# inferflow/inferflow

Measured on AMD Instinct MI355X. Metric: decode tokens/sec, Llama-2-7B Q4 batch=1 greedy (whole job), higher is better.
Workload: dtype i8 (Q8 activations x Q4_B32T1A weights, i32 dot, f32 scale, f16 I/O); 1 GPU; llama2_7b decode, Q4_B32T1A weights + F16 lm_head, F16 KV cache, batch 1 greedy, 16-token prompt, context 21..1851; parallelism=single, weights_bytes=4309647360

## Files before the change

### inferflow_amd/csrc/ifa_decode_attn.h

```cpp
#pragma once
#include "ifa_decode_kernels.h"

namespace ifa {

struct DecAttnParams {
    const half_t *q;
    const half_t *k_new;
    const half_t *v_new;
    uint8_t *kcache, *vcache;
    const int *state;
    const float *rope_tab;
    int heads, kv_heads, kv_q8;
    float kq_scale;
    int rope_order, rope_cols;
    int alibi, alibi_base, alibi_total;
    half_t *out;
    int max_ctx;
    int8_t *xq;
    long long *trace;
    const void *batch_rows;
    int q_stride;
};
struct DecAttnBatchRow { const uint8_t *kc, *vc; int n_ctx, pad; };

// ... 49 lines not shown
        if constexpr (IFA_ATTN_NACC == 1) return c[0];
        else if constexpr (IFA_ATTN_NACC == 2) return c[0] + c[1];
        else if constexpr (IFA_ATTN_NACC == 4) return (c[0] + c[1]) + (c[2] + c[3]);
        else { float t = c[0]; for (int i = 1; i < IFA_ATTN_NACC; i++) t = t + c[i]; return t; }
    }
};

struct DecAttnFusedIn {
    const unsigned long long *gran;
    unsigned epoch;
    int pos;
    unsigned *err;
    long long timeout_ticks;
    unsigned long long *att_gran;
};

__host__ __device__ inline int att_gran_count(int heads, int hd) { return heads * hd / 4 + 2 * (heads * hd / 32) + heads; }

template <int HD, bool Q8, int PB, bool KT>
struct DecAttnRegs {
    static constexpr int DG = HD / 8, NSPLIT = 256 / DG, VPRE = PB / NSPLIT;
    static constexpr int KBYTES = (HD / 32) * 34;
    static constexpr int KALIGN = HD == 128 ? 8 : (HD == 64 ? 4 : 2);
    uint32_t kreg[Q8 ? 1 : HD / 2];
    uint32_t kq32[(Q8 && KALIGN >= 4) ? KBYTES / 4 : 1];
    uint16_t kq16[(Q8 && KALIGN < 4) ? KBYTES / 2 : 1];
    u32x4 kt[KT ? PB / NSPLIT : 1];
    u32x4 vreg[Q8 ? 1 : VPRE];
    uint32_t vqs[Q8 ? VPRE : 1], vqc[Q8 ? VPRE : 1][2];
    float rope_cs, rope_sn;
    half_t q_in, k_in, v_in;
};

template <int HD, bool Q8, bool BATCH, int PB, bool KT, bool FUSED, int PHASE = 0>
__device__ __forceinline__ void dec_attn_body(char *smem, const half_t *pq, const uint8_t *pkc, const uint8_t *pvc, int pheads, int pkvh,
                                              const DecAttnParams &P, const int h_in, const DecAttnFusedIn &F, DecAttnRegs<HD, Q8, PB, KT> &R)
{
    int pos_b = 0;
    if constexpr (FUSED) pos_b = F.pos;
    if constexpr (BATCH) {
        const DecAttnBatchRow br = reinterpret_cast<const DecAttnBatchRow *>(P.batch_rows)[blockIdx.y];
        pkc = br.kc; pvc = br.vc; pos_b = br.n_ctx - 1;
        pq += (size_t)blockIdx.y * P.q_stride;
    }
#define IFA_GP(T, p) ((const __attribute__((address_space(1))) T *)(p))
    uint8_t *const kcw = BATCH ? const_cast<uint8_t *>(pkc) : P.kcache;
    uint8_t *const vcw = BATCH ? const_cast<uint8_t *>(pvc) : P.vcache;
    const float *const rope_tab = BATCH ? P.rope_tab + (size_t)blockIdx.y * HD : P.rope_tab;
    half_t *const outp = BATCH ? P.out + (size_t)blockIdx.y * pheads * HD : P.out;
    static_assert(HD % 8 == 0 && HD <= 128 && (!Q8 || HD % 32 == 0), "head size: multiples of 8 up to 128 (Q8 rows: whole 32-blocks)");
    constexpr int DG = HD / 8;
    constexpr int NSPLIT = 256 / DG;
    half_t *qs = reinterpret_cast<half_t *>(smem);
    half_t *kn = qs + HD;
    half_t *vn = kn + HD;
    float *red = reinterpret_cast<float *>(vn + HD);
    float *opart = red + 16;
    static_assert(!KT || (!Q8 && !BATCH && (DG & (DG - 1)) == 0 && PB % NSPLIT == 0), "K tile through LDS: F16 rows, one query, power-of-two pieces per row");
    static_assert(!(FUSED && BATCH), "the fused tail is a single-query kernel");
    static_assert(PB >= NSPLIT && PB <= DEC_ATTN_MIN_ROWS, "prefetch bucket");
    uint8_t *ktile = reinterpret_cast<uint8_t *>(opart + NSPLIT * HD);
    half_t *S = reinterpret_cast<half_t *>(ktile + (KT ? (size_t)PB * HD * 2 : 0));
    const int h = h_in, tid = threadIdx.x, lane = tid & 63, wave = tid >> 6;
    const int group = pheads / pkvh;
    const int kvh = h / group;
    const bool writer = (h % group) == 0;
    const int kv_dim = pkvh * HD;
    const size_t row_bytes = Q8 ? (size_t)(kv_dim / 32) * 34 : (size_t)kv_dim * 2;
    const size_t head_off = Q8 ? (size_t)((kvh * HD) / 32) * 34 : (size_t)kvh * HD * 2;

    constexpr int KBYTES = (HD / 32) * 34;
    constexpr int KALIGN = HD == 128 ? 8 : (HD == 64 ? 4 : 2);
    auto &kreg = R.kreg; auto &kq32 = R.kq32; auto &kq16 = R.kq16; auto &kt = R.kt; auto &vreg = R.vreg; auto &vqs = R.vqs; auto &vqc = R.vqc;
    float &rope_cs = R.rope_cs, &rope_sn = R.rope_sn;
    half_t &q_in = R.q_in, &k_in = R.k_in, &v_in = R.v_in;
    auto load_k = [&](int j) {
        const uint8_t *rowp = pkc + (size_t)j * row_bytes + head_off;
        if constexpr (Q8) {
            if constexpr (KALIGN == 8) {
#pragma unroll
                for (int i = 0; i < KBYTES / 8; i++) {
                    const u32x2 t = IFA_GP(u32x2, rowp)[i];
                    kq32[2 * i] = t[0]; kq32[2 * i + 1] = t[1];
                }
            } else if constexpr (KALIGN == 4) {
#pragma unroll
                for (int i = 0; i < KBYTES / 4; i++) kq32[i] = IFA_GP(uint32_t, rowp)[i];
            } else {
#pragma unroll
                for (int i = 0; i < KBYTES / 2; i++) kq16[i] = IFA_GP(uint16_t, rowp)[i];
            }
        } else {
#pragma unroll
            for (int i = 0; i < HD / 8; i++) {
                const u32x4 t = IFA_GP(u32x4, rowp)[i];
                kreg[4 * i] = t[0]; kreg[4 * i + 1] = t[1]; kreg[4 * i + 2] = t[2]; kreg[4 * i + 3] = t[3];
            }
        }
    };
    auto kbyte = [&](int B) -> uint32_t {
        if constexpr (KALIGN >= 4) return (kq32[B >> 2] >> (8 * (B & 3))) & 0xFFu;
        else return (kq16[B >> 1] >> (8 * (B & 1))) & 0xFFu;
    };
    const int dq = min(tid, HD - 1);
    if constexpr (PHASE != 2) {
    q_in = (half_t)0; k_in = (half_t)0; v_in = (half_t)0;
    if constexpr (!FUSED) { q_in = pq[(size_t)h * HD + dq]; k_in = pq[(size_t)(pheads + kvh) * HD + dq]; v_in = pq[(size_t)(pheads + pkvh + kvh) * HD + dq]; }
    }
    const int dg = tid % DG, sp = tid / DG;
    const bool vact = (256 % DG == 0) || sp < NSPLIT;
    constexpr int VPRE = PB / NSPLIT;
    if constexpr (PHASE != 2) {
    if constexpr (KT) {
#pragma unroll
        for (int i = 0; i < PB / NSPLIT; i++) kt[i] = IFA_GP(u32x4, pkc + (size_t)min(sp + NSPLIT * i, FUSED ? min(pos_b, PB - 1) : PB - 1) * row_bytes + head_off)[dg];
    } else {
        load_k((BATCH || FUSED) ? min(tid, min(pos_b, PB - 1)) : min(tid, PB - 1));
    }
    rope_cs = 1.0f; rope_sn = 0.0f;
    {
        const int c = min(tid < HD / 2 ? tid : tid - HD / 2, HD / 2 - 1);
        const float *rt = rope_tab ? rope_tab : reinterpret_cast<const float *>(pq);
        typedef float f32x2 __attribute__((ext_vector_type(2)));
        const f32x2 cs = *IFA_GP(f32x2, rt + 2 * c);
        if (P.rope_order != 0) { rope_cs = cs[0]; rope_sn = cs[1]; }
    }
    const size_t vq_off = head_off + (size_t)(dg / 4) * 34;
#pragma unroll
    for (int i = 0; i < VPRE; i++) {
        const int j = min(sp + NSPLIT * i, BATCH ? pos_b : (FUSED ? min(pos_b, PB - 1) : PB - 1));
        if constexpr (!Q8) {
            vreg[i] = IFA_GP(u32x4, pvc + (size_t)j * row_bytes + head_off)[dg];
        } else {
            const auto *blk = IFA_GP(uint16_t, pvc + (size_t)j * row_bytes + vq_off);
            typedef uint32_t u32x2_a2 __attribute__((ext_vector_type(2), aligned(2)));
            vqs[i] = blk[0];
            const u32x2_a2 cw = *IFA_GP(u32x2_a2, blk + 1 + (dg % 4) * 4);
            vqc[i][0] = cw[0]; vqc[i][1] = cw[1];
        }
    }
    }
    if constexpr (PHASE == 1) return;

    const bool tr = P.trace != nullptr && tid == 0;
    if (tr) P.trace[h * 8 + 0] = wall_clock64();
    const int pos = (BATCH || FUSED) ? pos_b : *(const __attribute__((address_space(4))) int *)(P.state + 1);
    const int n_ctx = pos + 1;
    if constexpr (FUSED) {
        if (tid < HD) {
            const unsigned long long *gq = F.gran + (size_t)h * HD + tid, *gk = F.gran + (size_t)(pheads + kvh) * HD + tid,
                                     *gv = F.gran + (size_t)(pheads + pkvh + kvh) * HD + tid;
            const long long t_give_up = wall_clock64() + F.timeout_ticks;
            for (;;) {
                const unsigned long long a = __hip_atomic_load(gq, __ATOMIC_RELAXED, __HIP_MEMORY_SCOPE_AGENT);
                const unsigned long long b = __hip_atomic_load(gk, __ATOMIC_RELAXED, __HIP_MEMORY_SCOPE_AGENT);
                const unsigned long long c = __hip_atomic_load(gv, __ATOMIC_RELAXED, __HIP_MEMORY_SCOPE_AGENT);
                const bool ok = (unsigned)(a >> 32) == F.epoch && (unsigned)(b >> 32) == F.epoch && (unsigned)(c >> 32) == F.epoch;
                q_in = __builtin_bit_cast(half_t, (uint16_t)a); k_in = __builtin_bit_cast(half_t, (uint16_t)b); v_in = __builtin_bit_cast(half_t, (uint16_t)c);
                if (__all(ok)) break;
                if (wall_clock64() > t_give_up) { if (lane == 0) atomicExch(F.err, 0x51u); break; }
                __builtin_amdgcn_s_sleep(2);
            }
        }
    }
    if (tid < HD) { qs[tid] = q_in; kn[tid] = k_in; vn[tid] = v_in; }
    if constexpr (KT) {
#pragma unroll
        for (int i = 0; i < PB / NSPLIT; i++) {
            const int j = sp + NSPLIT * i;
            *reinterpret_cast<u32x4 *>(ktile + ((size_t)j * DG + (size_t)(dg ^ (j & (DG - 1)))) * 16) = kt[i];
        }
    }
    __syncthreads();
    if (tr) P.trace[h * 8 + 1] = wall_clock64();
    if (P.rope_order != 0) {
        if (tid < HD) {
            const int c = tid < HD / 2 ? tid : tid - HD / 2;
            rope_apply(tid < HD / 2 ? qs : kn, c, rope_cs, rope_sn, P.rope_order, P.rope_cols);
        }
        __syncthreads();
    }
// ... 160 lines not shown
    __syncthreads();
    }
    if (tr) P.trace[h * 8 + 5] = wall_clock64();

    float o[8];
#pragma unroll
    for (int i = 0; i < 8; i++) o[i] = 0.0f;
    auto acc_v = [&](float pj, const u32x4 vv) {
        const half8_t v8 = __builtin_bit_cast(half8_t, vv);
#pragma unroll
        for (int e = 0; e < 8; e++) o[e] = __builtin_fmaf(pj, (float)v8[e], o[e]);
    };
    auto acc_new = [&](float pj) {
#pragma unroll
        for (int e = 0; e < 8; e++) o[e] = __builtin_fmaf(pj, h2f(vn[dg * 8 + e]), o[e]);
    };
    auto acc_q8w = [&](float pj, uint16_t scb, uint16_t c0, uint16_t c1, uint16_t c2, uint16_t c3) {
        const half_t sch = __builtin_bit_cast(half_t, scb);
        const half2_t sc2 = {sch, sch};
        half2_t v01, v23, v45, v67;
        q8x4_dequant_h((uint32_t)c0 | ((uint32_t)c1 << 16), sc2, v01, v23);
        q8x4_dequant_h((uint32_t)c2 | ((uint32_t)c3 << 16), sc2, v45, v67);
        o[0] = __builtin_fmaf(pj, (float)v01[0], o[0]); o[1] = __builtin_fmaf(pj, (float)v01[1], o[1]);
        o[2] = __builtin_fmaf(pj, (float)v23[0], o[2]); o[3] = __builtin_fmaf(pj, (float)v23[1], o[3]);
        o[4] = __builtin_fmaf(pj, (float)v45[0], o[4]); o[5] = __builtin_fmaf(pj, (float)v45[1], o[5]);
        o[6] = __builtin_fmaf(pj, (float)v67[0], o[6]); o[7] = __builtin_fmaf(pj, (float)v67[1], o[7]);
    };
    auto acc_q8 = [&](float pj, int j) {
        const auto *blk = IFA_GP(uint16_t, pvc + (size_t)j * row_bytes + head_off + (size_t)(dg / 4) * 34);
        typedef uint32_t u32x2_a2 __attribute__((ext_vector_type(2), aligned(2)));
        const u32x2_a2 cw = *IFA_GP(u32x2_a2, blk + 1 + (dg % 4) * 4);
        acc_q8w(pj, blk[0], (uint16_t)(cw[0] & 0xFFFFu), (uint16_t)(cw[0] >> 16), (uint16_t)(cw[1] & 0xFFFFu), (uint16_t)(cw[1] >> 16));
    };
#pragma unroll
    for (int i = 0; i < VPRE; i++) {
        const int j = sp + NSPLIT * i;
        if (j < n_ctx && vact) {
            const float pj = h2f(S[j]);
            if (j == pos) acc_new(pj);
            else if constexpr (Q8) acc_q8w(pj, (uint16_t)vqs[i], (uint16_t)(vqc[i][0] & 0xFFFFu), (uint16_t)(vqc[i][0] >> 16), (uint16_t)(vqc[i][1] & 0xFFFFu), (uint16_t)(vqc[i][1] >> 16));
            else acc_v(pj, vreg[i]);
        }
    }
    {
        constexpr int TB = 8;
        u32x4 tcur[Q8 ? 1 : TB], tnxt[Q8 ? 1 : TB];
        uint32_t ts_c[Q8 ? TB : 1], tc_c[Q8 ? TB : 1][2], ts_n[Q8 ? TB : 1], tc_n[Q8 ? TB : 1][2];
        const size_t tq_off = head_off + (size_t)(dg / 4) * 34;
        auto tload = [&](u32x4 (&dst)[Q8 ? 1 : TB], uint32_t (&ds)[Q8 ? TB : 1], uint32_t (&dc)[Q8 ? TB : 1][2], int j) {
#pragma unroll
            for (int u = 0; u < TB; u++) {
                const int jr = min(j + u * NSPLIT, n_ctx - 1);
                if constexpr (!Q8) dst[u] = IFA_GP(u32x4, pvc + (size_t)jr * row_bytes + head_off)[dg];
                else {
                    const auto *blk = IFA_GP(uint16_t, pvc + (size_t)jr * row_bytes + tq_off);
                    typedef uint32_t u32x2_a2 __attribute__((ext_vector_type(2), aligned(2)));
                    ds[u] = blk[0];
                    const u32x2_a2 cw = *IFA_GP(u32x2_a2, blk + 1 + (dg % 4) * 4);
                    dc[u][0] = cw[0]; dc[u][1] = cw[1];
                }
            }
        };
        int j = vact ? sp + NSPLIT * VPRE : n_ctx;
        if (j < n_ctx) tload(tcur, ts_c, tc_c, j);
        for (; j < n_ctx; j += TB * NSPLIT) {
            tload(tnxt, ts_n, tc_n, j + TB * NSPLIT);
#pragma unroll
            for (int u = 0; u < TB; u++) {
                const int jj = j + u * NSPLIT;
                if (jj >= n_ctx) break;
                const float pj = h2f(S[jj]);
                if (jj == pos) acc_new(pj);
                else if constexpr (Q8) acc_q8w(pj, (uint16_t)ts_c[u], (uint16_t)(tc_c[u][0] & 0xFFFFu), (uint16_t)(tc_c[u][0] >> 16), (uint16_t)(tc_c[u][1] & 0xFFFFu), (uint16_t)(tc_c[u][1] >> 16));
                else acc_v(pj, tcur[u]);
            }
#pragma unroll
            for (int u = 0; u < TB; u++) {
                if constexpr (Q8) { ts_c[u] = ts_n[u]; tc_c[u][0] = tc_n[u][0]; tc_c[u][1] = tc_n[u][1]; }
                else tcur[u] = tnxt[u];
            }
        }
    }
    if (vact) {
#pragma unroll
        for (int e = 0; e < 8; e++) opart[sp * HD + dg * 8 + e] = o[e];
    }
    if (tr) P.trace[h * 8 + 6] = wall_clock64();
    __syncthreads();
    if (tid < HD) {
        float acc = opart[tid];
        for (int s2 = 1; s2 < NSPLIT; s2++) acc = acc + opart[s2 * HD + tid];
        const half_t yh = f2h(acc);
        outp[(size_t)h * HD + tid] = yh;
        if constexpr (HD % 32 == 0 && !BATCH) { if (P.xq) dec_attn_emit_q8<HD>(P.xq, P.heads * HD, h, tid, yh); }
        if constexpr (FUSED && HD % 32 == 0) {
            if (F.att_gran) {
                const float val = h2f(yh);
                const float mxv = half_wave_max(fabsf(val));
                const float qsc = mxv / 127;
                const int qv = q8_round_div1(val, qsc);
                const int sum = half_wave_sum_i32(qv);
                const int q1 = dpp_xor1(qv), q2 = dpp_xor2(qv), q3 = dpp_xor1(q2);
                const unsigned long long tagw = (unsigned long long)F.epoch << 32;
                const int cols = pheads * HD, nc = cols / 4, nbk = cols / 32;
                if ((tid & 3) == 0) {
                    const uint32_t w4 = (uint32_t)(qv & 0xFF) | ((uint32_t)(q1 & 0xFF) << 8) | ((uint32_t)(q2 & 0xFF) << 16) | ((uint32_t)(q3 & 0xFF) << 24);
                    __hip_atomic_store(F.att_gran + (h * HD + tid) / 4, tagw | w4, __ATOMIC_RELAXED, __HIP_MEMORY_SCOPE_AGENT);
                }
                if ((tid & 31) == 0) {
                    const int blk = (h * HD + tid) >> 5;
                    __hip_atomic_store(F.att_gran + nc + blk, tagw | __builtin_bit_cast(uint32_t, h2f(f2h(qsc))), __ATOMIC_RELAXED, __HIP_MEMORY_SCOPE_AGENT);
                    __hip_atomic_store(F.att_gran + nc + nbk + blk, tagw | __builtin_bit_cast(uint32_t, (float)sum), __ATOMIC_RELAXED, __HIP_MEMORY_SCOPE_AGENT);
                }
                if (tid == 0) __hip_atomic_store(F.att_gran + nc + 2 * nbk + h, tagw | 1u, __ATOMIC_RELAXED, __HIP_MEMORY_SCOPE_AGENT);
            }
        }
    }
    if (tr) P.trace[h * 8 + 7] = wall_clock64();
}

template <int HD, bool Q8, bool BATCH = false, int PB = DEC_ATTN_MIN_ROWS, bool KT = false>
__global__ void __launch_bounds__(256) k_dec_attn(const half_t *pq, const uint8_t *pkc, const uint8_t *pvc, int pheads, int pkvh,
                                                  const DecAttnParams P)
{
// ... 341 lines not shown
```

### inferflow_amd/csrc/ifa_decode_qkv_attn.h

```cpp
#pragma once
#include "ifa_decode_kernels.h"
#include "ifa_decode_attn.h"

namespace ifa {

struct DecQkvAttnExtra {
    unsigned long long *gran;
    const unsigned *epoch;
    unsigned epoch_add;
    unsigned *err;
    int timeout_us;
    int gk;
    int unload;
};

#ifndef IFA_QA_EARLY_KV
#define IFA_QA_EARLY_KV 0
#endif
#ifndef IFA_QA_WARM_ROWS
#define IFA_QA_WARM_ROWS 1
#endif
constexpr int QA_THREADS = 512;

template <int DT, int NJ, int RW, int NORM, int HD, bool Q8, int PB, bool KT, int NP, bool UL = false>
__global__ void __launch_bounds__(QA_THREADS) k_dec_qkv_attn(const half_t *px, const half_t *pnw, const half_t *pnb, int pcols, int pgeo,
                                                             const uint8_t *pwq, const uint8_t *pwk, const uint8_t *pwv,
                                                             const DecGemvParams P, const DecAttnParams A, const DecQkvAttnExtra E)
{
    const int g_heads = pgeo & 0xFF, g_kvh = (pgeo >> 8) & 0xFF, g_gk = (pgeo >> 16) & 0xFFFF;
    const int g_nblk = pcols / block_capacity(DT);
    extern __shared__ __attribute__((aligned(16))) char smem[];
    const long long t_kernel = wall_clock64();
    static_assert(NORM == 0 || NORM == 1, "QKV prologue: quantiser with or without the RMS norm");
    static_assert(NP > 0 && NP * 64 < QA_THREADS, "wave-specialised prologue");
    constexpr int TH = QA_THREADS, PT = NP * 64;
    constexpr int MAXC = (NJ * 8 * block_capacity(DT) + PT - 1) / PT;
    XPre<NORM, MAXC, false, PT> pre;
    if (threadIdx.x < PT) pre.issue(px, pnw, pnb, pcols);
    const XLds L = xlds_carve(smem, pcols);
    const int lane = threadIdx.x & 63;
    const int wave = __builtin_amdgcn_readfirstlane(threadIdx.x >> 6);
    using Fmt = DecFmt<DT, NJ>;
    const size_t row_bytes = tiled_row_bytes(DT, (size_t)g_nblk);
    const int g = (int)blockIdx.x / g_gk, bg = (int)blockIdx.x - g * g_gk;
    const int group = g_heads / g_kvh;
    const int RG = (group + 2) * HD;
    const int per = g_gk / group;
    const bool attn_wg = bg % per == 0;
    const int head = g * group + bg / per;
    const int WGV = UL ? (g_gk - group) * (TH / 64) : g_gk * (TH / 64);
    const int lw = UL ? (bg - bg / per - 1) * (TH / 64) + wave : bg * (TH / 64) + wave;
    struct Row { const uint8_t *w; const half_t *b; half_t *y; int row, vrow; };
    auto locate = [&](int lr) {
        Row r;
        const int nq = group * HD;
        const bool isk = lr >= nq && lr < nq + HD, isv = lr >= nq + HD;
        r.row = isv ? g * HD + (lr - nq - HD) : (isk ? g * HD + (lr - nq) : g * nq + lr);
// ... 27 lines not shown
    };
    static_assert(NP == 4, "the prologue waves are the attention waves");
    const bool ul_head = UL && attn_wg;
    if (!ul_head && threadIdx.x == TH - 1) { L.part[130] = 0.0f; L.part[131] = 0.0f; }
    if (!ul_head && wave >= NP) load_rows(0, 1);
    const int pos = *(const __attribute__((address_space(4))) int *)(A.state + 1);
    const unsigned epoch = ((*(const __attribute__((address_space(4))) unsigned *)(E.epoch) + E.epoch_add) << 20) | ((unsigned)pos & 0xFFFFFu);
    DecAttnFusedIn F;
    F.gran = E.gran; F.epoch = epoch; F.pos = pos; F.err = E.err; F.timeout_ticks = (long long)E.timeout_us * 100;
    F.att_gran = nullptr;
    if constexpr (UL) {
        if (attn_wg) {
            if (wave >= 4) {
#if IFA_QA_WARM_ROWS
                if (pos >= PB) {
                    constexpr int SB = Q8 ? (HD / 32) * 34 : HD * 2;
                    const int kvh = head / group, kv_dim = g_kvh * HD;
                    const size_t rb = Q8 ? (size_t)(kv_dim / 32) * 34 : (size_t)kv_dim * 2;
                    const size_t ho = Q8 ? (size_t)((kvh * HD) / 32) * 34 : (size_t)kvh * HD * 2;
                    const int t = (int)threadIdx.x - 256;
                    const int off = min((t & 3) * 64, SB - 4) & ~1;
                    typedef uint32_t u32_a2 __attribute__((aligned(2)));
                    uint32_t acc = 0;
                    for (int j = PB + (t >> 2); j <= pos; j += 64) {
                        acc ^= *(const __attribute__((address_space(1))) u32_a2 *)(A.kcache + (size_t)j * rb + ho + off);
                        acc ^= *(const __attribute__((address_space(1))) u32_a2 *)(A.vcache + (size_t)j * rb + ho + off);
                    }
                    if (acc == 0x9E3779B9u && A.trace) A.trace[(size_t)A.heads * 8 + 7] = (long long)acc;
                }
#endif
                return;
            }
            DecAttnRegs<HD, Q8, PB, KT> RU;
            dec_attn_body<HD, Q8, false, PB, KT, true>(smem, nullptr, A.kcache, A.vcache, A.heads, A.kv_heads, A, head, F, RU);
            return;
        }
    }
    __syncthreads();
    DecAttnRegs<HD, Q8, PB, KT> R;
    if (wave >= NP) {
        load_rows(1, RW);
    } else {
        pre.finish(P.norm_w, P.norm_b, P.multi_base, P.eps, P.cols, L, P.xn_out, nullptr);
        load_rows(0, RW);
#if IFA_QA_EARLY_KV
        if (attn_wg) dec_attn_body<HD, Q8, false, PB, KT, true, 1>(smem, nullptr, A.kcache, A.vcache, A.heads, A.kv_heads, A, head, F, R);
#endif
    }
    lds_counter_wait(L.part + 131, NP);
    typename Fmt::X X;
    X.load(L.codes, L.scale, L.xsum, lane, g_nblk);
    {
        float a[RW];
#pragma unroll
        for (int i = 0; i < RW; i++) a[i] = w[i].dot(X);
#pragma unroll
        for (int i = 0; i < RW; i++) a[i] = wave_sum(a[i]);
        float a0 = 0.0f;
#pragma unroll
        for (int i = 0; i < RW; i++) { if (lane == i) a0 = a[i]; }
        const int lr = lane * WGV + lw;
        if (lane < RW && lr < RG) {
            const Row r = locate(lr);
            half_t y = dec_bias(a0, r.b, r.row);
            if (P.pre_scale != 0.0f) y = f2h(h2f(y) * P.pre_scale);
            r.y[r.row] = y;
            __hip_atomic_store(E.gran + r.vrow, ((unsigned long long)epoch << 32) | (unsigned long long)__builtin_bit_cast(uint16_t, y),
                               __ATOMIC_RELAXED, __HIP_MEMORY_SCOPE_AGENT);
        }
    }
    if (A.trace && threadIdx.x == 0) {
        A.trace[(size_t)(A.heads + (int)blockIdx.x) * 8 + 0] = t_kernel;
        A.trace[(size_t)(A.heads + (int)blockIdx.x) * 8 + 1] = wall_clock64();
    }
    if (attn_wg) {
        __syncthreads();
        if (wave >= 4) return;
        dec_attn_body<HD, Q8, false, PB, KT, true, IFA_QA_EARLY_KV ? 2 : 0>(smem, nullptr, A.kcache, A.vcache, A.heads, A.kv_heads, A, head, F, R);
        return;
    }
}

bool dec_qkv_attn_supported(int w_dtype, int cols, int heads, int kv_heads, int head_dim, int num_cus, int *gk_out, int *rw_out);
int dec_qkv_attn_launch(int w_dtype, int norm, bool kv_q8, int pb, bool kt, const DecGemvParams &P, const DecAttnParams &A, const DecQkvAttnExtra &E,
                        int max_ctx, hipStream_t s);
template <int DT>
int dec_qkv_attn_launch_dt(int norm, bool kv_q8, int pb, bool kt, int rw, const DecGemvParams &P, const DecAttnParams &A, const DecQkvAttnExtra &E,
                           int max_ctx, hipStream_t s);

}
```

### inferflow_amd/csrc/ifa_dqkvattn_impl.h

```cpp
#pragma once
#include "ifa_host.h"
#include "ifa_decode_qkv_attn.h"

namespace ifa {

template <int DT, int NJ, int RW, int NORM, bool Q8, int PB, bool KT, bool UL = false>
static int qa_go(const DecGemvParams &P, const DecAttnParams &A, const DecQkvAttnExtra &E, int max_ctx, hipStream_t s)
{
    constexpr int HD = 128;
    auto kern = k_dec_qkv_attn<DT, NJ, RW, NORM, HD, Q8, PB, KT, QA_THREADS / 128, UL>;
    const size_t smem = std::max(xlds_bytes(P.cols), dec_attn_smem(HD, max_ctx, KT ? PB : 0));
    if (smem > (size_t)160 * 1024) return ifa_fail(IFA_ERR_ARG, "fused QKV + attention: %zu bytes of LDS", smem);
    if (smem > 48 * 1024) IFA_HIP_CHECK(hipFuncSetAttribute((const void *)kern, hipFuncAttributeMaxDynamicSharedMemorySize, (int)smem));
    if (A.heads > 255 || A.kv_heads > 255 || E.gk > 0xFFFF) return ifa_fail(IFA_ERR_ARG, "fused QKV + attention: geometry exceeds the packed launch scalar");
    const int pgeo = A.heads | (A.kv_heads << 8) | (E.gk << 16);
    kern<<<dim3((unsigned)(A.kv_heads * E.gk)), dim3(QA_THREADS), smem, s>>>(P.x, P.norm_w, P.norm_b, P.cols, pgeo, P.W0[0], P.W0[1], P.W0[2], P, A, E);
    IFA_LAUNCH_CHECK();
    return IFA_OK;
}

template <int DT, int NJ, int RW, int NORM>
static int qa_pick(bool kv_q8, int pb, bool kt, const DecGemvParams &P, const DecAttnParams &A, const DecQkvAttnExtra &E, int max_ctx, hipStream_t s)
{
    if (kv_q8) {
        if (pb == 64) return qa_go<DT, NJ, RW, NORM, true, 64, false>(P, A, E, max_ctx, s);
        if (pb == 128) return qa_go<DT, NJ, RW, NORM, true, 128, false>(P, A, E, max_ctx, s);
        return qa_go<DT, NJ, RW, NORM, true, 256, false>(P, A, E, max_ctx, s);
    }
    if (kt) {
        if (pb == 64) return qa_go<DT, NJ, RW, NORM, false, 64, true>(P, A, E, max_ctx, s);
        if (pb == 128) return qa_go<DT, NJ, RW, NORM, false, 128, true>(P, A, E, max_ctx, s);
        return qa_go<DT, NJ, RW, NORM, false, 256, true>(P, A, E, max_ctx, s);
    }
    return qa_go<DT, NJ, RW, NORM, false, 256, false>(P, A, E, max_ctx, s);
}

template <int DT, int NJ, int RW, int NORM>
static int qa_pick_ul(bool kv_q8, int pb, bool kt, const DecGemvParams &P, const DecAttnParams &A, const DecQkvAttnExtra &E, int max_ctx, hipStream_t s)
{
    if (pb == 128) {
        if (kv_q8) return qa_go<DT, NJ, RW, NORM, true, 128, false, true>(P, A, E, max_ctx, s);
        if (kt) return qa_go<DT, NJ, RW, NORM, false, 128, true, true>(P, A, E, max_ctx, s);
    }
    if (kv_q8) return qa_go<DT, NJ, RW, NORM, true, 256, false, true>(P, A, E, max_ctx, s);
    if (kt) return qa_go<DT, NJ, RW, NORM, false, 256, true, true>(P, A, E, max_ctx, s);
    return qa_go<DT, NJ, RW, NORM, false, 256, false, true>(P, A, E, max_ctx, s);
}

template <int DT> constexpr int qa_nj(int cols) { return (cols / block_capacity(DT) + 63) / 64; }

template <int DT>
// ... 15 lines not shown
```

### inferflow_amd/csrc/ifa_engine.hip

```cpp
#include "ifa_engine_state.h"

namespace ifae {

int perf_begin(ifa_model *m, int key)
{
    if (!m->opt_perf_stat) return -1;
    hipStreamCaptureStatus cs = hipStreamCaptureStatusNone;
    if (hipStreamIsCapturing(m->stream, &cs) != hipSuccess || cs != hipStreamCaptureStatusNone) { (void)hipGetLastError(); return -1; }
    auto take = [&]() -> hipEvent_t {
        if (!m->perf_pool.empty()) { hipEvent_t e = m->perf_pool.back(); m->perf_pool.pop_back(); return e; }
        hipEvent_t e = nullptr;
        if (hipEventCreate(&e) != hipSuccess) { (void)hipGetLastError(); return nullptr; }
        return e;
    };
    ifa_model::PerfSpanRec r; r.key = key; r.e0 = take(); r.e1 = take();
    if (!r.e0 || !r.e1) { if (r.e0) m->perf_pool.push_back(r.e0); if (r.e1) m->perf_pool.push_back(r.e1); return -1; }
    if (hipEventRecord(r.e0, m->stream) != hipSuccess) { (void)hipGetLastError(); m->perf_pool.push_back(r.e0); m->perf_pool.push_back(r.e1); return -1; }
    m->perf_spans.push_back(r);
    return (int)m->perf_spans.size() - 1;
}

void perf_end(ifa_model *m, int idx)
{
    if (idx < 0 || idx >= (int)m->perf_spans.size()) return;
// ... 471 lines not shown
    }
    IFA_HIP_CHECK(hipStreamSynchronize(m->stream));
    return IFA_OK;
}

int ifa_model_select_kv(ifa_model *m, int slot)
{
    IFA_REQUIRE(m && m->finalized, "ifa_model_select_kv: model not finalized");
    if (m->slots.empty()) m->slots.resize(1);
    IFA_REQUIRE(slot >= 0 && slot < (int)m->slots.size(), "ifa_model_select_kv: slot %d of %zu", slot, m->slots.size());
    if (slot == m->cur_slot) return IFA_OK;
    if (m->tp_graph_exec) { (void)hipGraphExecDestroy(m->tp_graph_exec); m->tp_graph_exec = nullptr; }
    if (m->tp_graph) { (void)hipGraphDestroy(m->tp_graph); m->tp_graph = nullptr; }
    ifa_model::KvSlot &out = m->slots[(size_t)m->cur_slot], &in = m->slots[(size_t)slot];
    out.k.clear(); out.v.clear();
    for (Layer &L : m->layers) { out.k.push_back(L.kcache); out.v.push_back(L.vcache); }
    out.graph = m->graph; out.exec = m->graph_exec;
    if (m->graph_exec_n) { (void)hipGraphExecDestroy(m->graph_exec_n); m->graph_exec_n = nullptr; }
    if (m->graph_n) { (void)hipGraphDestroy(m->graph_n); m->graph_n = nullptr; }
    for (size_t l = 0; l < m->layers.size(); l++) { m->layers[l].kcache = in.k[l]; m->layers[l].vcache = in.v[l]; }
    m->graph = in.graph; m->graph_exec = in.exec;
    in.k.clear(); in.v.clear(); in.graph = nullptr; in.exec = nullptr;
    m->cur_slot = slot;
    return IFA_OK;
}

int ifa_model_set_option(ifa_model *m, const char *name, int value)
{
    IFA_REQUIRE(m && name, "ifa_model_set_option: null pointer");
    if (strcmp(name, "pool_lse") == 0) { m->opt_pool_lse = value != 0; return IFA_OK; }
    struct { const char *n; int *p; } opts[] = {
        {"fused", &m->opt_fused}, {"graph", &m->opt_graph}, {"rpw_qkv", &m->opt_rpw_qkv}, {"rpw_wo", &m->opt_rpw_wo},
        {"rpw_ffn", &m->opt_rpw_ffn}, {"rpw_w2", &m->opt_rpw_w2}, {"rpw_lm", &m->opt_rpw_lm}, {"trace", &m->opt_trace},
        {"bench_mode", &m->opt_bench_mode}, {"touch_stride", &m->opt_touch_stride}, {"attn_split_ctx", &m->opt_attn_split_ctx}, {"batch_graph", &m->opt_batch_graph}, {"gemm_rows", &m->opt_gemm_rows}, {"batch_fused", &m->opt_batch_fused}, {"rows_mo", &m->opt_rows_mo}, {"debug_mo_alloc_fail", &m->opt_debug_mo_alloc_fail}, {"rows_kparts", &m->opt_rows_kparts}, {"prefill_chunk", &m->opt_prefill_chunk}, {"prefill_big_min", &m->opt_prefill_big_min}, {"prefill_mid", &m->opt_prefill_mid}, {"prefill_mid_max", &m->opt_prefill_mid_max}, {"prefill_res_mid", &m->opt_prefill_res_mid}, {"gemm_splitk", &m->opt_gemm_splitk}, {"moe_singles", &m->opt_moe_singles}, {"moe_overlap", &m->opt_moe_overlap}, {"prefill_big", &m->opt_prefill_big}, {"moe_router_fused", &m->opt_moe_router_fused}, {"tp_fuse_add", &m->opt_tp_fuse_add}, {"attn_q8", &m->opt_attn_q8}, {"attn_kt", &m->opt_attn_kt}, {"fuse_attn", &m->opt_fuse_attn}, {"fuse_ffn", &m->opt_fuse_ffn}, {"attn_post_as_residual", &m->opt_attn_post_as_residual}, {"chain_late_w2", &m->opt_chain_late_w2}, {"exact_order", &m->opt_exact_order}, {"perf_stat", &m->opt_perf_stat}, {"attn_nsplits", &m->opt_attn_nsplits}, {"attn_unload", &m->opt_attn_unload}, {"q3h_native", &m->opt_q3h_native}, {"fuse_attn_timeout_us", &m->opt_fuse_attn_timeout_us}, {"step_tail", &m->opt_step_tail}, {"graph_steps", &m->opt_graph_steps}, {"moe_device", &m->opt_moe_device}, 
        
        {"debug_layers", &m->opt_debug_layers}, {"debug_layer0", &m->opt_debug_layer0}, {"debug_hidden_in", &m->opt_debug_hidden_in}};
    for (auto &o : opts)
        if (strcmp(o.n, name) == 0) {
            *o.p = value;
            drop_graphs(m);
            return IFA_OK;
        }
    return ifa_fail(IFA_ERR_ARG, "ifa_model_set_option: unknown option '%s'", name);
}

int ifa_model_perf_stat(ifa_model *m, int *keys_out, float *ms_out, int cap, int *n_out, int clear)
{
    IFA_REQUIRE(m && n_out && cap >= 0 && (cap == 0 || (keys_out && ms_out)), "ifa_model_perf_stat: null pointer");
    IFA_HIP_CHECK(hipSetDevice(m->cfg.device));
    int rc = perf_collect(m);
    if (rc) return rc;
    int n = 0;
    for (auto &kv : m->perf_map) {
        if (n < cap) { keys_out[n] = kv.first; ms_out[n] = kv.second; }
        n++;
    }
    *n_out = n;
    if (clear) m->perf_map.clear();
    return IFA_OK;
}

int ifa_model_set_excluded_tokens(ifa_model *m, const int *ids_host, int n)
{
    IFA_REQUIRE(m && m->finalized, "ifa_model_set_excluded_tokens: model not finalized");
    IFA_REQUIRE(n >= 0 && n <= 3 && (n == 0 || ids_host), "ifa_model_set_excluded_tokens: n %d (0..3)", n);
    int v[4] = {n, -1, -1, -1};
    for (int i = 0; i < n; i++) v[1 + i] = ids_host[i];
// ... 87 lines not shown
```

### inferflow_amd/csrc/ifa_engine_decode.hip

```cpp
#include "ifa_engine_state.h"

namespace ifae {

bool qkv_attn_layer_ok(const ifa_model *m, int l, int *gk_out);

static int attn_split_threshold(const ifa_model *m)
{
    if (m->opt_attn_split_ctx >= 0) return m->opt_attn_split_ctx;
    const ifa_model_config &c = m->cfg;
    bool tail = m->opt_attn_unload && m->opt_fuse_attn && waits_enabled() && dec_attn_smem(c.head_dim, c.max_ctx, 256) <= IFA_LDS_LIMIT;
    int gk = 0;
    for (int l = 0; tail && l < c.layers; l++) if (!qkv_attn_layer_ok(m, l, &gk)) tail = false;
    if (tail && (long long)c.kv_heads * gk > (long long)visible_cus()) tail = false;
    if (!tail) return 320;
    return c.heads > c.kv_heads ? 640 : 512;
}

void choose_attn_split(ifa_model *m, int reach)
{
    const int thr = attn_split_threshold(m);
    const int want = (thr > 0 && reach > thr) ? (reach > 8192 ? 16 : 8) : 0;
    if (want != m->attn_split) { m->attn_split = want; drop_graphs(m); }
    const int pb = reach <= 64 ? 64 : (reach <= 128 ? 128 : 256);
    if (pb != m->attn_pb) { m->attn_pb = pb; drop_graphs(m); }
// ... 190 lines not shown
    return IFA_OK;
}

void qkv_params(ifa_model *m, int l, const half_t *x, DecGemvParams &P)
{
    const ifa_model_config &c = m->cfg;
    Layer &L = m->layers[(size_t)l];
    memset(&P, 0, sizeof(P));
    P.x = x; P.norm_w = (const half_t *)L.t[T_ATTN_NORM].data; P.norm_b = (const half_t *)L.t[T_ATTN_NORM_B].data;
    P.multi_base = c.attn_norm_base; P.eps = c.eps; P.cols = c.dim; P.nblk = c.dim / 32;
    if (c.parallel_attn) P.xn_out = m->xn;
    const int ids[3] = {T_WQ, T_WK, T_WV}; const int bids[3] = {T_WQ_B, T_WK_B, T_WV_B};
    const size_t QDd = (size_t)c.heads * c.head_dim, KVDd = (size_t)c.kv_heads * c.head_dim;
    half_t *outs[3] = {m->dqkv, m->dqkv + QDd, m->dqkv + QDd + KVDd};
    for (int i = 0; i < 3; i++) {
        P.W0[i] = wbytes(L.t[ids[i]]); P.b0[i] = (const half_t *)L.t[bids[i]].data;
        P.y[i] = outs[i]; P.rows[i] = (int)L.t[ids[i]].rows;
    }
    P.nsets = 3;
}

int launch_qkv_attn(ifa_model *m, int l, const half_t *x, unsigned tag_add)
{
    const ifa_model_config &c = m->cfg;
    Layer &L = m->layers[(size_t)l];
    DecGemvParams P; qkv_params(m, l, x, P);
    DecAttnParams A; attn_params(m, l, A);
    DecQkvAttnExtra E; memset(&E, 0, sizeof(E));
    E.gran = m->qa_gran + (size_t)l * (size_t)(c.heads + 2 * c.kv_heads) * c.head_dim;
    E.epoch = m->qa_call; E.epoch_add = tag_add; E.err = m->qa_err; E.timeout_us = m->opt_fuse_attn_timeout_us; E.gk = m->qa_gk;
    const int pb = (m->attn_pb == 64 || m->attn_pb == 128) ? m->attn_pb : 256;
    const bool kt = m->opt_attn_kt && !A.kv_q8 && dec_attn_smem(c.head_dim, c.max_ctx, pb) <= IFA_LDS_LIMIT;
    E.unload = ((m->opt_attn_unload >= 1 && pb == 256) || (m->opt_attn_unload >= 2 && pb == 128 && (kt || A.kv_q8))) ? 1 : 0;
    return dec_qkv_attn_launch(L.t[T_WQ].dtype, 1, A.kv_q8 != 0, pb, kt, P, A, E, c.max_ctx, m->stream);
}

int launch_qkv(ifa_model *m, int l, const half_t *x)
{
    const ifa_model_config &c = m->cfg;
    Layer &L = m->layers[(size_t)l];
    DecGemvParams P; memset(&P, 0, sizeof(P));
    P.x = x; P.norm_w = (const half_t *)L.t[T_ATTN_NORM].data; P.norm_b = (const half_t *)L.t[T_ATTN_NORM_B].data;
    P.multi_base = c.attn_norm_base; P.eps = c.eps; P.cols = c.dim; P.nblk = c.dim / 32;
    if (c.parallel_attn) P.xn_out = m->xn;
    const bool std_norm = c.norm_kind != 0;
    if (std_norm) {
        int rc = sep_norm(m, x, L.t[T_ATTN_NORM], L.t[T_ATTN_NORM_B], m->xn);
        if (rc) return rc;
        P.x = m->xn; P.norm_w = nullptr; P.norm_b = nullptr; P.xn_out = nullptr;
    }
    const int ids[3] = {T_WQ, T_WK, T_WV}; const int bids[3] = {T_WQ_B, T_WK_B, T_WV_B};
    const size_t QDd = (size_t)c.heads * c.head_dim, KVDd = (size_t)c.kv_heads * c.head_dim;
    half_t *outs[3] = {m->dqkv, m->dqkv + QDd, m->dqkv + QDd + KVDd};
    for (int i = 0; i < 3; i++) {
        P.W0[i] = wbytes(L.t[ids[i]]); P.b0[i] = (const half_t *)L.t[bids[i]].data;
        P.y[i] = outs[i]; P.rows[i] = (int)L.t[ids[i]].rows;
    }
    P.nsets = 3;
    if (m->pend.on && !std_norm) {
        P.x = m->pend.x; P.x_add = m->pend.add; P.x_add_bias = m->pend.bias; P.xsum_out = m->pend.out;
        m->pend.on = false;
    }
    auto go = [&](int dtype, const DecGemvParams &Q) {
        if (std_norm) return launch_dec_gemv<EPI_PLAIN, 0>(dtype, Q, m->opt_rpw_qkv, m->stream);
        return launch_dec_gemv<EPI_PLAIN, 1>(dtype, Q, m->opt_rpw_qkv, m->stream);
    };
// ... 586 lines not shown
```

### inferflow_amd/csrc/ifa_engine_state.h

```cpp
#pragma once
#include <chrono>
#include <cstdlib>
#include <cstring>
#include <map>
#include <string>
#include <vector>
#include "ifa_host.h"
#include "ifa_decode_kernels.h"
#include "ifa_decode_attn.h"
#include "ifa_decode_gemv.h"
#include "ifa_moe.h"
#include "ifa_gemm_rows_mfma.h"
#include "ifa_gemm_big.h"
#include "ifa_decode_lmhead_tail.h"
#include "ifa_decode_singles.h"
#include "ifa_decode_qkv_attn.h"
#include "ifa_decode_chain.h"

using namespace ifa;

namespace ifae {


enum { T_EMBD = 0, T_OUT_NORM = 1, T_OUT_NORM_B = 2, T_LM_HEAD = 3,
// ... 40 lines not shown
    half_t *bqkv = nullptr;
    float *brope = nullptr;
    size_t bqkv_rows = 0;
    half_t *att = nullptr, *a = nullptr, *f = nullptr, *t1 = nullptr, *t2 = nullptr, *logits = nullptr;
    uint8_t *xq = nullptr;
    int8_t *attq = nullptr;
    half_t *moe_gate = nullptr, *moe_out = nullptr;
    half_t *moe_in = nullptr, *moe_wdev = nullptr;
    int *moe_route = nullptr;
    int *moe_idx = nullptr, *moe_pin = nullptr;
    int *moe_sel = nullptr, *moe_epos = nullptr, *moe_counts = nullptr;
    half_t *moe_selw = nullptr, *moe_g1 = nullptr, *moe_g3 = nullptr, *moe_gin = nullptr, *moe_gout = nullptr;
    uint8_t *moe_xq_in = nullptr, *moe_xq_mid = nullptr;
    void *moe_tiles = nullptr, *moe_singles = nullptr, *moe_smalls = nullptr;
    int opt_moe_device = 1;
    int *state = nullptr;
    float *rope_tab = nullptr;
    long long *trace = nullptr;
    int opt_trace = 0, opt_bench_mode = 0, opt_touch_stride = 65536;
    int *tokens_dev = nullptr;
    int *host_pinned = nullptr;
    int scratch_tokens = 0;
    size_t kv_row_bytes = 0;
    hipGraph_t graph = nullptr;
    hipGraphExec_t graph_exec = nullptr;
    hipGraph_t graph_n = nullptr; hipGraphExec_t graph_exec_n = nullptr; int graph_n_steps = 0, opt_graph_steps = 1;
    struct PendingAdd { const half_t *x = nullptr, *add = nullptr, *bias = nullptr; half_t *out = nullptr; bool on = false; } pend;
    int opt_tp_fuse_add = 1;
    void *batch_tab_dev = nullptr, *batch_tab_pin = nullptr;
    size_t batch_tab_bytes = 0;
    std::map<int, hipGraphExec_t> batch_graphs;
    DecAttnSplitWs attn_ws = {nullptr, nullptr, nullptr, 8};
    int opt_attn_unload = 1;
    int opt_attn_nsplits = 0;
    int opt_fuse_attn = 1, opt_fuse_attn_timeout_us = 20000, qa_on = 0, qa_gk = 0;
    unsigned long long *qa_gran = nullptr;
    unsigned *qa_call = nullptr, *qa_err = nullptr, qa_calls = 0;
    int opt_fuse_ffn = 0, ch_on = 0, opt_chain_late_w2 = 0;
    int opt_q3h_native = 0;
    int opt_perf_stat = 0;
    struct PerfSpanRec { int key; hipEvent_t e0, e1; };
    std::vector<PerfSpanRec> perf_spans;
    std::vector<hipEvent_t> perf_pool;
    std::map<int, float> perf_map;
    int opt_exact_order = 0;
    float *exact_rope_tab = nullptr;
    uint32_t *ch_gran = nullptr, *ch_flags = nullptr;
    int opt_step_tail = 1, st_on = 0;
    unsigned long long *st_keys = nullptr; unsigned *st_counter = nullptr; int st_keys_n = 0;
    int attn_pb = 256, opt_attn_kt = 1;
    int attn_split = 0, opt_attn_split_ctx = -1, opt_batch_graph = 0, opt_gemm_rows = 1, opt_batch_fused = 1, opt_moe_router_fused = 1, opt_prefill_big = 1, opt_rows_mo = 1, opt_moe_singles = 1;
    struct KvSlot { std::vector<void *> k, v; hipGraph_t graph = nullptr; hipGraphExec_t exec = nullptr; };
    std::vector<KvSlot> slots;
    int cur_slot = 0;
    int opt_attn_q8 = 1;
    half_t *tp_a = nullptr, *tp_f = nullptr, *tp_hid = nullptr, *tp_logits = nullptr;
    float *tp_best = nullptr, *tp_gather = nullptr;
    int *tp_tok = nullptr;
    hipGraph_t tp_graph = nullptr;
    hipGraphExec_t tp_graph_exec = nullptr;
    struct TpKey {
        unsigned long long tp = 0, world = 0; int tp_size = 0, stage = 0, n_stages = 0, prev = 0, next = 0, src = 0, voff = 0, force = 0, fuse = 0, slot = 0, oneshot = 0;
        bool operator==(const TpKey &o) const { return tp == o.tp && world == o.world && tp_size == o.tp_size && stage == o.stage && n_stages == o.n_stages
                && prev == o.prev && next == o.next && src == o.src && voff == o.voff && force == o.force && fuse == o.fuse && slot == o.slot
                && oneshot == o.oneshot; }
    } tp_key;
// ... 193 lines not shown
```

Baseline: 625.0 tokens/s.

## Add short-tail variant of fused QKV+attention with early granule loads

Adds a TAIL template path to the fused QKV+attention kernel, on by default through a new attn_tail option. It issues the granule atomic loads for q/k/v early, before the K/V prefetch, so their latency overlaps other work. The V accumulation is restructured so the P values are gathered up front and the newly produced V row is substituted from LDS instead of taking a separate branch. The final split reduction is unrolled into registers. The cost is more template instantiations and register pressure, plus a spin loop that now polls preloaded values.

```diff
diff --git a/inferflow_amd/csrc/ifa_decode_attn.h b/inferflow_amd/csrc/ifa_decode_attn.h
--- a/inferflow_amd/csrc/ifa_decode_attn.h
+++ b/inferflow_amd/csrc/ifa_decode_attn.h
@@ -105,7 +105,7 @@
     half_t q_in, k_in, v_in;
 };
 
-template <int HD, bool Q8, bool BATCH, int PB, bool KT, bool FUSED, int PHASE = 0>
+template <int HD, bool Q8, bool BATCH, int PB, bool KT, bool FUSED, int PHASE = 0, bool TAIL = false>
 __device__ __forceinline__ void dec_attn_body(char *smem, const half_t *pq, const uint8_t *pkc, const uint8_t *pvc, int pheads, int pkvh,
                                               const DecAttnParams &P, const int h_in, const DecAttnFusedIn &F, DecAttnRegs<HD, Q8, PB, KT> &R)
 {
@@ -131,6 +131,7 @@
     float *opart = red + 16;
     static_assert(!KT || (!Q8 && !BATCH && (DG & (DG - 1)) == 0 && PB % NSPLIT == 0), "K tile through LDS: F16 rows, one query, power-of-two pieces per row");
     static_assert(!(FUSED && BATCH), "the fused tail is a single-query kernel");
+    static_assert(!TAIL || FUSED, "the short tail is a form of the fused launch");
     static_assert(PB >= NSPLIT && PB <= DEC_ATTN_MIN_ROWS, "prefetch bucket");
     uint8_t *ktile = reinterpret_cast<uint8_t *>(opart + NSPLIT * HD);
     half_t *S = reinterpret_cast<half_t *>(ktile + (KT ? (size_t)PB * HD * 2 : 0));
@@ -180,6 +181,13 @@
     q_in = (half_t)0; k_in = (half_t)0; v_in = (half_t)0;
     if constexpr (!FUSED) { q_in = pq[(size_t)h * HD + dq]; k_in = pq[(size_t)(pheads + kvh) * HD + dq]; v_in = pq[(size_t)(pheads + pkvh + kvh) * HD + dq]; }
     }
+    unsigned long long g_q = 0, g_k = 0, g_v = 0;
+    auto gran_load = [&]() {
+        g_q = __hip_atomic_load(F.gran + (size_t)h * HD + dq, __ATOMIC_RELAXED, __HIP_MEMORY_SCOPE_AGENT);
+        g_k = __hip_atomic_load(F.gran + (size_t)(pheads + kvh) * HD + dq, __ATOMIC_RELAXED, __HIP_MEMORY_SCOPE_AGENT);
+        g_v = __hip_atomic_load(F.gran + (size_t)(pheads + pkvh + kvh) * HD + dq, __ATOMIC_RELAXED, __HIP_MEMORY_SCOPE_AGENT);
+    };
+    if constexpr (TAIL && PHASE == 0) gran_load();
     const int dg = tid % DG, sp = tid / DG;
     const bool vact = (256 % DG == 0) || sp < NSPLIT;
     constexpr int VPRE = PB / NSPLIT;
@@ -219,7 +227,20 @@
     if (tr) P.trace[h * 8 + 0] = wall_clock64();
     const int pos = (BATCH || FUSED) ? pos_b : *(const __attribute__((address_space(4))) int *)(P.state + 1);
     const int n_ctx = pos + 1;
-    if constexpr (FUSED) {
+    if constexpr (TAIL) {
+        if constexpr (PHASE != 0) gran_load();
+        if (tid < HD) {
+            const long long t_give_up = wall_clock64() + F.timeout_ticks;
+            for (;;) {
+                const bool ok = (unsigned)(g_q >> 32) == F.epoch && (unsigned)(g_k >> 32) == F.epoch && (unsigned)(g_v >> 32) == F.epoch;
+                q_in = __builtin_bit_cast(half_t, (uint16_t)g_q); k_in = __builtin_bit_cast(half_t, (uint16_t)g_k); v_in = __builtin_bit_cast(half_t, (uint16_t)g_v);
+                if (__all(ok)) break;
+                if (wall_clock64() > t_give_up) { if (lane == 0) atomicExch(F.err, 0x51u); break; }
+                __builtin_amdgcn_s_sleep(2);
+                gran_load();
+            }
+        }
+    } else if constexpr (FUSED) {
         if (tid < HD) {
             const unsigned long long *gq = F.gran + (size_t)h * HD + tid, *gk = F.gran + (size_t)(pheads + kvh) * HD + tid,
                                      *gv = F.gran + (size_t)(pheads + pkvh + kvh) * HD + tid;
@@ -446,6 +467,31 @@
         const u32x2_a2 cw = *IFA_GP(u32x2_a2, blk + 1 + (dg % 4) * 4);
         acc_q8w(pj, blk[0], (uint16_t)(cw[0] & 0xFFFFu), (uint16_t)(cw[0] >> 16), (uint16_t)(cw[1] & 0xFFFFu), (uint16_t)(cw[1] >> 16));
     };
+    if constexpr (TAIL) {
+        const u32x4 vnew = *reinterpret_cast<const u32x4 *>(vn + (vact ? dg * 8 : 0));
+        float pjs[VPRE];
+#pragma unroll
+        for (int i = 0; i < VPRE; i++) pjs[i] = h2f(S[min(sp + NSPLIT * i, pos)]);
+#pragma unroll
+        for (int i = 0; i < VPRE; i++) {
+            const int j = sp + NSPLIT * i;
+            u32x4 vv;
+            if constexpr (Q8) {
+                const half_t sch = __builtin_bit_cast(half_t, (uint16_t)vqs[i]);
+                const half2_t sc2 = {sch, sch};
+                half2_t v01, v23, v45, v67;
+                q8x4_dequant_h(vqc[i][0], sc2, v01, v23);
+                q8x4_dequant_h(vqc[i][1], sc2, v45, v67);
+                vv[0] = __builtin_bit_cast(uint32_t, v01); vv[1] = __builtin_bit_cast(uint32_t, v23);
+                vv[2] = __builtin_bit_cast(uint32_t, v45); vv[3] = __builtin_bit_cast(uint32_t, v67);
+            } else {
+                vv = vreg[i];
+            }
+            const bool isnew = j == pos;
+            vv[0] = isnew ? vnew[0] : vv[0]; vv[1] = isnew ? vnew[1] : vv[1]; vv[2] = isnew ? vnew[2] : vv[2]; vv[3] = isnew ? vnew[3] : vv[3];
+            if (j < n_ctx && vact) acc_v(pjs[i], vv);
+        }
+    } else {
 #pragma unroll
     for (int i = 0; i < VPRE; i++) {
         const int j = sp + NSPLIT * i;
@@ -455,6 +501,7 @@
             else if constexpr (Q8) acc_q8w(pj, (uint16_t)vqs[i], (uint16_t)(vqc[i][0] & 0xFFFFu), (uint16_t)(vqc[i][0] >> 16), (uint16_t)(vqc[i][1] & 0xFFFFu), (uint16_t)(vqc[i][1] >> 16));
             else acc_v(pj, vreg[i]);
         }
+    }
     }
     {
         constexpr int TB = 8;
@@ -502,8 +549,18 @@
     if (tr) P.trace[h * 8 + 6] = wall_clock64();
     __syncthreads();
     if (tid < HD) {
-        float acc = opart[tid];
-        for (int s2 = 1; s2 < NSPLIT; s2++) acc = acc + opart[s2 * HD + tid];
+        float acc;
+        if constexpr (TAIL) {
+            float part[NSPLIT];
+#pragma unroll
+            for (int s2 = 0; s2 < NSPLIT; s2++) part[s2] = opart[s2 * HD + tid];
+            acc = part[0];
+#pragma unroll
+            for (int s2 = 1; s2 < NSPLIT; s2++) acc = acc + part[s2];
+        } else {
+            acc = opart[tid];
+            for (int s2 = 1; s2 < NSPLIT; s2++) acc = acc + opart[s2 * HD + tid];
+        }
         const half_t yh = f2h(acc);
         outp[(size_t)h * HD + tid] = yh;
         if constexpr (HD % 32 == 0 && !BATCH) { if (P.xq) dec_attn_emit_q8<HD>(P.xq, P.heads * HD, h, tid, yh); }
diff --git a/inferflow_amd/csrc/ifa_decode_qkv_attn.h b/inferflow_amd/csrc/ifa_decode_qkv_attn.h
--- a/inferflow_amd/csrc/ifa_decode_qkv_attn.h
+++ b/inferflow_amd/csrc/ifa_decode_qkv_attn.h
@@ -12,6 +12,7 @@
     int timeout_us;
     int gk;
     int unload;
+    int tail;
 };
 
 #ifndef IFA_QA_EARLY_KV
@@ -22,7 +23,7 @@
 #endif
 constexpr int QA_THREADS = 512;
 
-template <int DT, int NJ, int RW, int NORM, int HD, bool Q8, int PB, bool KT, int NP, bool UL = false>
+template <int DT, int NJ, int RW, int NORM, int HD, bool Q8, int PB, bool KT, int NP, bool UL = false, bool TAIL = false>
 __global__ void __launch_bounds__(QA_THREADS) k_dec_qkv_attn(const half_t *px, const half_t *pnw, const half_t *pnb, int pcols, int pgeo,
                                                              const uint8_t *pwq, const uint8_t *pwk, const uint8_t *pwv,
                                                              const DecGemvParams P, const DecAttnParams A, const DecQkvAttnExtra E)
@@ -116,7 +117,7 @@
                 return;
             }
             DecAttnRegs<HD, Q8, PB, KT> RU;
-            dec_attn_body<HD, Q8, false, PB, KT, true>(smem, nullptr, A.kcache, A.vcache, A.heads, A.kv_heads, A, head, F, RU);
+            dec_attn_body<HD, Q8, false, PB, KT, true, 0, TAIL>(smem, nullptr, A.kcache, A.vcache, A.heads, A.kv_heads, A, head, F, RU);
             return;
         }
     }
@@ -128,7 +129,7 @@
         pre.finish(P.norm_w, P.norm_b, P.multi_base, P.eps, P.cols, L, P.xn_out, nullptr);
         load_rows(0, RW);
 #if IFA_QA_EARLY_KV
-        if (attn_wg) dec_attn_body<HD, Q8, false, PB, KT, true, 1>(smem, nullptr, A.kcache, A.vcache, A.heads, A.kv_heads, A, head, F, R);
+        if (attn_wg) dec_attn_body<HD, Q8, false, PB, KT, true, 1, TAIL>(smem, nullptr, A.kcache, A.vcache, A.heads, A.kv_heads, A, head, F, R);
 #endif
     }
     lds_counter_wait(L.part + 131, NP);
@@ -160,7 +161,7 @@
     if (attn_wg) {
         __syncthreads();
         if (wave >= 4) return;
-        dec_attn_body<HD, Q8, false, PB, KT, true, IFA_QA_EARLY_KV ? 2 : 0>(smem, nullptr, A.kcache, A.vcache, A.heads, A.kv_heads, A, head, F, R);
+        dec_attn_body<HD, Q8, false, PB, KT, true, IFA_QA_EARLY_KV ? 2 : 0, TAIL>(smem, nullptr, A.kcache, A.vcache, A.heads, A.kv_heads, A, head, F, R);
         return;
     }
 }
diff --git a/inferflow_amd/csrc/ifa_dqkvattn_impl.h b/inferflow_amd/csrc/ifa_dqkvattn_impl.h
--- a/inferflow_amd/csrc/ifa_dqkvattn_impl.h
+++ b/inferflow_amd/csrc/ifa_dqkvattn_impl.h
@@ -4,11 +4,11 @@
 
 namespace ifa {
 
-template <int DT, int NJ, int RW, int NORM, bool Q8, int PB, bool KT, bool UL = false>
-static int qa_go(const DecGemvParams &P, const DecAttnParams &A, const DecQkvAttnExtra &E, int max_ctx, hipStream_t s)
+template <int DT, int NJ, int RW, int NORM, bool Q8, int PB, bool KT, bool UL, bool TAIL>
+static int qa_go2(const DecGemvParams &P, const DecAttnParams &A, const DecQkvAttnExtra &E, int max_ctx, hipStream_t s)
 {
     constexpr int HD = 128;
-    auto kern = k_dec_qkv_attn<DT, NJ, RW, NORM, HD, Q8, PB, KT, QA_THREADS / 128, UL>;
+    auto kern = k_dec_qkv_attn<DT, NJ, RW, NORM, HD, Q8, PB, KT, QA_THREADS / 128, UL, TAIL>;
     const size_t smem = std::max(xlds_bytes(P.cols), dec_attn_smem(HD, max_ctx, KT ? PB : 0));
     if (smem > (size_t)160 * 1024) return ifa_fail(IFA_ERR_ARG, "fused QKV + attention: %zu bytes of LDS", smem);
     if (smem > 48 * 1024) IFA_HIP_CHECK(hipFuncSetAttribute((const void *)kern, hipFuncAttributeMaxDynamicSharedMemorySize, (int)smem));
@@ -17,6 +17,13 @@
     kern<<<dim3((unsigned)(A.kv_heads * E.gk)), dim3(QA_THREADS), smem, s>>>(P.x, P.norm_w, P.norm_b, P.cols, pgeo, P.W0[0], P.W0[1], P.W0[2], P, A, E);
     IFA_LAUNCH_CHECK();
     return IFA_OK;
+}
+
+template <int DT, int NJ, int RW, int NORM, bool Q8, int PB, bool KT, bool UL = false>
+static int qa_go(const DecGemvParams &P, const DecAttnParams &A, const DecQkvAttnExtra &E, int max_ctx, hipStream_t s)
+{
+    if (E.tail) return qa_go2<DT, NJ, RW, NORM, Q8, PB, KT, UL, true>(P, A, E, max_ctx, s);
+    return qa_go2<DT, NJ, RW, NORM, Q8, PB, KT, UL, false>(P, A, E, max_ctx, s);
 }
 
 template <int DT, int NJ, int RW, int NORM>
diff --git a/inferflow_amd/csrc/ifa_engine.hip b/inferflow_amd/csrc/ifa_engine.hip
--- a/inferflow_amd/csrc/ifa_engine.hip
+++ b/inferflow_amd/csrc/ifa_engine.hip
@@ -527,7 +527,7 @@
     struct { const char *n; int *p; } opts[] = {
         {"fused", &m->opt_fused}, {"graph", &m->opt_graph}, {"rpw_qkv", &m->opt_rpw_qkv}, {"rpw_wo", &m->opt_rpw_wo},
         {"rpw_ffn", &m->opt_rpw_ffn}, {"rpw_w2", &m->opt_rpw_w2}, {"rpw_lm", &m->opt_rpw_lm}, {"trace", &m->opt_trace},
-        {"bench_mode", &m->opt_bench_mode}, {"touch_stride", &m->opt_touch_stride}, {"attn_split_ctx", &m->opt_attn_split_ctx}, {"batch_graph", &m->opt_batch_graph}, {"gemm_rows", &m->opt_gemm_rows}, {"batch_fused", &m->opt_batch_fused}, {"rows_mo", &m->opt_rows_mo}, {"debug_mo_alloc_fail", &m->opt_debug_mo_alloc_fail}, {"rows_kparts", &m->opt_rows_kparts}, {"prefill_chunk", &m->opt_prefill_chunk}, {"prefill_big_min", &m->opt_prefill_big_min}, {"prefill_mid", &m->opt_prefill_mid}, {"prefill_mid_max", &m->opt_prefill_mid_max}, {"prefill_res_mid", &m->opt_prefill_res_mid}, {"gemm_splitk", &m->opt_gemm_splitk}, {"moe_singles", &m->opt_moe_singles}, {"moe_overlap", &m->opt_moe_overlap}, {"prefill_big", &m->opt_prefill_big}, {"moe_router_fused", &m->opt_moe_router_fused}, {"tp_fuse_add", &m->opt_tp_fuse_add}, {"attn_q8", &m->opt_attn_q8}, {"attn_kt", &m->opt_attn_kt}, {"fuse_attn", &m->opt_fuse_attn}, {"fuse_ffn", &m->opt_fuse_ffn}, {"attn_post_as_residual", &m->opt_attn_post_as_residual}, {"chain_late_w2", &m->opt_chain_late_w2}, {"exact_order", &m->opt_exact_order}, {"perf_stat", &m->opt_perf_stat}, {"attn_nsplits", &m->opt_attn_nsplits}, {"attn_unload", &m->opt_attn_unload}, {"q3h_native", &m->opt_q3h_native}, {"fuse_attn_timeout_us", &m->opt_fuse_attn_timeout_us}, {"step_tail", &m->opt_step_tail}, {"graph_steps", &m->opt_graph_steps}, {"moe_device", &m->opt_moe_device}, 
+        {"bench_mode", &m->opt_bench_mode}, {"touch_stride", &m->opt_touch_stride}, {"attn_split_ctx", &m->opt_attn_split_ctx}, {"batch_graph", &m->opt_batch_graph}, {"gemm_rows", &m->opt_gemm_rows}, {"batch_fused", &m->opt_batch_fused}, {"rows_mo", &m->opt_rows_mo}, {"debug_mo_alloc_fail", &m->opt_debug_mo_alloc_fail}, {"rows_kparts", &m->opt_rows_kparts}, {"prefill_chunk", &m->opt_prefill_chunk}, {"prefill_big_min", &m->opt_prefill_big_min}, {"prefill_mid", &m->opt_prefill_mid}, {"prefill_mid_max", &m->opt_prefill_mid_max}, {"prefill_res_mid", &m->opt_prefill_res_mid}, {"gemm_splitk", &m->opt_gemm_splitk}, {"moe_singles", &m->opt_moe_singles}, {"moe_overlap", &m->opt_moe_overlap}, {"prefill_big", &m->opt_prefill_big}, {"moe_router_fused", &m->opt_moe_router_fused}, {"tp_fuse_add", &m->opt_tp_fuse_add}, {"attn_q8", &m->opt_attn_q8}, {"attn_kt", &m->opt_attn_kt}, {"fuse_attn", &m->opt_fuse_attn}, {"fuse_ffn", &m->opt_fuse_ffn}, {"attn_post_as_residual", &m->opt_attn_post_as_residual}, {"chain_late_w2", &m->opt_chain_late_w2}, {"exact_order", &m->opt_exact_order}, {"perf_stat", &m->opt_perf_stat}, {"attn_nsplits", &m->opt_attn_nsplits}, {"attn_unload", &m->opt_attn_unload}, {"attn_tail", &m->opt_attn_tail}, {"q3h_native", &m->opt_q3h_native}, {"fuse_attn_timeout_us", &m->opt_fuse_attn_timeout_us}, {"step_tail", &m->opt_step_tail}, {"graph_steps", &m->opt_graph_steps}, {"moe_device", &m->opt_moe_device}, 
         
         {"debug_layers", &m->opt_debug_layers}, {"debug_layer0", &m->opt_debug_layer0}, {"debug_hidden_in", &m->opt_debug_hidden_in}};
     for (auto &o : opts)
diff --git a/inferflow_amd/csrc/ifa_engine_decode.hip b/inferflow_amd/csrc/ifa_engine_decode.hip
--- a/inferflow_amd/csrc/ifa_engine_decode.hip
+++ b/inferflow_amd/csrc/ifa_engine_decode.hip
@@ -246,6 +246,7 @@
     const int pb = (m->attn_pb == 64 || m->attn_pb == 128) ? m->attn_pb : 256;
     const bool kt = m->opt_attn_kt && !A.kv_q8 && dec_attn_smem(c.head_dim, c.max_ctx, pb) <= IFA_LDS_LIMIT;
     E.unload = ((m->opt_attn_unload >= 1 && pb == 256) || (m->opt_attn_unload >= 2 && pb == 128 && (kt || A.kv_q8))) ? 1 : 0;
+    E.tail = m->opt_attn_tail;
     return dec_qkv_attn_launch(L.t[T_WQ].dtype, 1, A.kv_q8 != 0, pb, kt, P, A, E, c.max_ctx, m->stream);
 }
 
diff --git a/inferflow_amd/csrc/ifa_engine_state.h b/inferflow_amd/csrc/ifa_engine_state.h
--- a/inferflow_amd/csrc/ifa_engine_state.h
+++ b/inferflow_amd/csrc/ifa_engine_state.h
@@ -96,6 +96,7 @@
     std::map<int, hipGraphExec_t> batch_graphs;
     DecAttnSplitWs attn_ws = {nullptr, nullptr, nullptr, 8};
     int opt_attn_unload = 1;
+    int opt_attn_tail = 1;
     int opt_attn_nsplits = 0;
     int opt_fuse_attn = 1, opt_fuse_attn_timeout_us = 20000, qa_on = 0, qa_gk = 0;
     unsigned long long *qa_gran = nullptr;
```

Measured after the change: 626.0 tokens/s, median of 3. Within noise of the previous version (+0.2%).
